# monahand1023/imageclust

Hardware: AMD Instinct MI355X
Metric: images/sec (embed+Ward) (higher is better)
Workload: dtype bf16; 1 GPU; the metric's size (configs[2]'s N=100000) on 1 GPU: 100000 synthetic 224x224x3 images (structured, seed 20250217; 100000 on this rank), ResNet50-v1 bf16 batch=256 -> 2048-d pooled E -> Ward min=5 max=50 (merge loop on GPU0) -> cluster ids on host; n_images_total=100000, embed_dim=2048, weights=synthetic seed 1, device=AMD Radeon Graphics (gfx950:sramecc+:xnack-)

## Files before the change

### imageclust_amd/_lib.py

```python
import ctypes as C
import os

import numpy as np

_HERE = os.path.dirname(os.path.abspath(__file__))
SO_PATH = os.environ.get("ICL_SO_PATH") or os.path.join(_HERE, "libimageclust_hip.so")

ICL_OK = 0
ICL_ERR_ARG, ICL_ERR_CONSTRAINT, ICL_ERR_HIP, ICL_ERR_NOMODEL, ICL_ERR_IO, ICL_ERR_UNSUPPORTED, ICL_ERR_OVERSIZE, ICL_ERR_NOMEM = range(1, 9)
HEAD_POOLED, HEAD_DENSE0 = 2048, 1000
PREC_FP32, PREC_BF16, PREC_BF16X3 = 0, 1, 2
UPDATE_EXACT, UPDATE_LW = 0, 1
SYNTH_NOISE, SYNTH_STRUCTURED = 0, 1
TILES_AUTO, TILES_LOCAL, TILES_DISTRIBUTED = 0, 1, 2
MERGE_GPU0, MERGE_SHARDED = 0, 1
CONV_P8_OFF, CONV_P8_AUTO, CONV_P8_ALL = 0, 1, 2
CONV_SPLIT = 16
ROWS_SINGLE, ROWS_EXACT_BATCH, ROWS_LW_BOUND, ROWS_LW_FAST, ROWS_SINGLE_APART = 0, 1, 2, 3, 4
FILE_FAIL_NEXT_LEADER = 0x100
MANY_MID_AUTO, MANY_MID_OFF, MANY_MID_ON = 0, 1, 2
PNG_HOST, PNG_GPU = 0, 1
ENTROPY_HOST, ENTROPY_GPU = 0, 1
K_CONV, K_DIST_EXACT, K_DIST_MFMA, K_ROWMIN, K_UPDATE, K_EMBED_OTHER, K_CONV64 = range(7)
K_NAMES = ["conv_igemm_kernel<*,128>", "ward_dist_exact_kernel", "dist_mfma_kernel", "row_argmin_*_kernel",
# ... 57 lines not shown
    ("icl_jpeg_coefs_mem", _int, [_vp, _vp, _vp, _i64, _int, _vp, _i64, _vp, _vp]),
    ("icl_jpeg_encode_bound", _i64, [_i32, _i32]),
    ("icl_jpeg_encode_rgb", _int, [_vp, _i32, _i32, _i32, _vp, _i64, _pi64]),
    ("icl_jpeg_encode_rgb_dev", _int, [_vp, _vp, _vp, _vp, _vp, _i64, _i32, _vp, _i32, _i64, _vp]),
    ("icl_downsize_image_file", _int, [C.c_char_p, _i64, _i32, _vp, _i64, _pi64, _vp]),
    ("icl_downsize_image_mem", _int, [_vp, _i64, _i64, _i32, _vp, _i64, _pi64, _vp]),
    ("icl_downsize_images", _int, [_vp, _vp, _i64, _i64, _i32, _i32, _vp, _i64, _vp, _vp]),
    ("icl_downsize_images_mem", _int, [_vp, _vp, _vp, _i64, _i64, _i32, _i32, _vp, _i64, _vp, _vp]),
    ("icl_last_downsize_stats", _int, [_vp, _pi64, _pi64, _pi64, _pi64, _pi64, _pi64, _vp]),
    ("icl_set_batch", _int, [_vp, _int]),
    ("icl_set_conv_options", _int, [_vp, _int]),
    ("icl_conv_stats", _int, [_vp, _vp, _vp]),
    ("icl_set_forward_prune", _int, [_vp, _int]),
    ("icl_forward_prune_stats", _int, [_vp, _vp]),
    ("icl_set_forward_prune_fused", _int, [_vp, _int]),
    ("icl_forward_prune_fused_stats", _int, [_vp, _vp]),
    ("icl_bottleneck56_sub", _int, [_vp, _vp, _int, _int, _int] + [_vp] * 9 + [_int, _int, _vp]),
    ("icl_conv1x1_mapped", _int, [_vp, _vp, _int, _int, _int, _int, _vp, _int, _vp, _vp, _vp, _int, _vp]),
    ("icl_conv_split_launches", _int, [_vp, _vp]),
    ("icl_conv2d_fused", _int, [_vp, _int, _vp, _int, _int, _int, _vp, _int, _int, _int, _int, _vp, _vp, _vp, _int, _vp]),
    ("icl_conv2d_dual", _int, [_vp, _int, _vp, _int, _int, _int, _vp, _vp, _int, _int, _vp, _int, _int, _vp, _vp, _int, _vp]),
    ("icl_embed_taps", _int, [_vp, _int, _vp, _int, _int, _vp]),
    ("icl_stem_pool", _int, [_vp, _int, _vp, _int, _vp]),
    ("icl_bottleneck56", _int, [_vp, _vp, _int, _int, _int, _int] + [_vp] * 13),
    ("icl_calc_optimal_clusters", _int, [_i64, _i64, _i64, _pi64]),
    ("icl_ward_distance_matrix", _int, [_vp, _vp, _vp, _i64, _i32, _vp, _i64]),
    ("icl_ward_distance_matrix_dev", _int, [_vp, _vp, _vp, _i64, _i32, _vp, _i64]),
    ("icl_merge_centroid", _int, [_vp, _vp, _i64, _vp, _i64, _i32, _vp]),
    ("icl_update_distance_matrix", _int, [_vp, _vp, _i64, _i64, _vp, _vp, _i32, _i64, _i64, _vp, _i64]),
    ("icl_find_closest", _int, [_vp, _vp, _i64, _i64, _pi64, _pi64]),
    ("icl_find_closest_dev", _int, [_vp, _vp, _i64, _i64, _pi64, _pi64]),
    ("icl_group_create", _int, [_pi32, _i32, C.POINTER(_vp)]),
    ("icl_group_destroy", None, [_vp]),
    ("icl_group_size", _i32, [_vp]),
    ("icl_group_ctx", _vp, [_vp, _i32]),
    ("icl_group_last_error", C.c_char_p, [_vp]),
    ("icl_group_load_onnx", _int, [_vp, C.c_char_p]),
    ("icl_group_load_blob", _int, [_vp, _vp, _i64]),
    ("icl_group_load_synthetic", _int, [_vp, C.c_uint64]),
    ("icl_group_embed_u8", _int, [_vp, _vp, _i64, _int, _int, _vp]),
    ("icl_group_cluster", _int, [_vp, _vp, _i64, _i32, _i32, _i32, _int, _vp, _vp, _pi32]),
    ("icl_set_ward_options", _int, [_vp, _int]),
    ("icl_embed_cluster_dev", _int, [_vp, _vp, _i64, _int, _i32, _i32, _int, _int, _vp, _vp, _vp, _pi32]),
    ("icl_group_embed_cluster", _int, [_vp, _vp, _i64, _int, _i32, _i32, _int, _vp, _vp, _vp, _pi32]),
    ("icl_ward_rows_partition", _int, [_i64, _i32, _i32, _pi64, _pi64]),
    ("icl_ward_span", _int, [_i64, _i64, _pi64, _pi64]),
# ... 473 lines not shown
        a, b = C.c_int64(0), C.c_int64(0)
        check(self.h, self.L.icl_conv_stats(self.h, C.byref(a), C.byref(b)))
        return a.value, b.value

    def conv_split_launches(self):
        a = C.c_int64(0)
        check(self.h, self.L.icl_conv_split_launches(self.h, C.byref(a)))
        return a.value

    def set_conv_options(self, p8_mode=1):
        check(self.h, self.L.icl_set_conv_options(self.h, p8_mode))

    def set_forward_prune(self, on=True):
        check(self.h, self.L.icl_set_forward_prune(self.h, 1 if on else 0))

    def forward_prune_stats(self):
        a = C.c_int64(0)
        check(self.h, self.L.icl_forward_prune_stats(self.h, C.byref(a)))
        return a.value

    def set_forward_prune_fused(self, on=True):
        check(self.h, self.L.icl_set_forward_prune_fused(self.h, 1 if on else 0))

    def forward_prune_fused_stats(self):
        a = C.c_int64(0)
        check(self.h, self.L.icl_forward_prune_fused_stats(self.h, C.byref(a)))
        return a.value

    def embed_u8(self, imgs, head=HEAD_POOLED, prec=PREC_FP32):
        imgs = np.ascontiguousarray(imgs, np.uint8).reshape(-1, IMG_BYTES)
        n = imgs.shape[0]
        out = np.empty((n, head), np.float32)
        check(self.h, self.L.icl_embed_u8(self.h, imgs.ctypes.data, n, head, prec, out.ctypes.data))
        return out

    def embed_u8_dev(self, d_imgs, n, d_out, head=HEAD_POOLED, prec=PREC_BF16):
        check(self.h, self.L.icl_embed_u8_dev(self.h, _vp(d_imgs), n, head, prec, _vp(d_out)))

    def embed_file(self, path, head=HEAD_DENSE0):
        out = np.empty(head, np.float32)
        check(self.h, self.L.icl_embed_file(self.h, os.fsencode(path), head, out.ctypes.data))
        return out

    def _files_call(self, fn, paths, *args):
        enc = [os.fsencode(p) for p in paths]
        arr = (C.c_char_p * max(1, len(enc)))(*enc)
# ... 242 lines not shown

    def conv2d_dual(self, x_nhwc, w1, x2_nhwc, w2, stride2, scale, shift, relu=True, prec=PREC_FP32):
        f = lambda a: np.ascontiguousarray(a, np.float32)
        x, x2, w1, w2, sc, sh = f(x_nhwc), f(x2_nhwc), f(w1), f(w2), f(scale), f(shift)
        B, Ho, _, Cin = x.shape
        _, H2, _, Cin2 = x2.shape
        Cout = w1.shape[0]
        assert x2.shape[0] == B and w1.shape == (Cout, Cin) and w2.shape == (Cout, Cin2) and sc.shape == (Cout,) and sh.shape == (Cout,)
        y = np.empty((B, Ho, Ho, Cout), np.float32)
        check(self.h, self.L.icl_conv2d_dual(self.h, prec, x.ctypes.data, B, Ho, Cin, w1.ctypes.data, x2.ctypes.data, H2, Cin2, w2.ctypes.data,
                                             int(stride2), Cout, sc.ctypes.data, sh.ctypes.data, 1 if relu else 0, y.ctypes.data))
        return y

    def embed_taps(self, imgs, tap, prec=PREC_FP32):
        a = np.ascontiguousarray(imgs, np.uint8).reshape(-1, IMG_BYTES)
        out = np.empty((a.shape[0],) + tap_shape(tap), np.float32)
        check(self.h, self.L.icl_embed_taps(self.h, prec, a.ctypes.data, a.shape[0], int(tap), out.ctypes.data))
        return out

    def stem_pool(self, imgs, prec=PREC_FP32):
        a = np.ascontiguousarray(imgs, np.uint8).reshape(-1, IMG_BYTES)
        out = np.empty((a.shape[0], 56, 56, 64), np.float32)
        check(self.h, self.L.icl_stem_pool(self.h, prec, a.ctypes.data, a.shape[0], out.ctypes.data))
        return out

    def bottleneck56(self, x_nhwc, w1, bn1, w2_oihw, bn2, w3, bn3, wds=None, bnds=None):
        f = lambda a: np.ascontiguousarray(a, np.float32)
        x = f(x_nhwc)
        B, H, W, Cin = x.shape
        y = np.empty((B, H, W, 256), np.float32)
        keep = [x, f(w1), f(bn1[0]), f(bn1[1]), f(w2_oihw), f(bn2[0]), f(bn2[1]), f(w3), f(bn3[0]), f(bn3[1])]
        keep += [None, None, None] if wds is None else [f(wds), f(bnds[0]), f(bnds[1])]
        ptr = [None if a is None else a.ctypes.data for a in keep]
        check(self.h, self.L.icl_bottleneck56(self.h, ptr[0], B, H, W, Cin, *ptr[1:], y.ctypes.data))
        return y

    def bottleneck56_sub(self, x_nhwc, w1, bn1, w2_oihw, bn2, w3, bn3, sub, fill):
        f = lambda a: np.ascontiguousarray(a, np.float32)
        x = f(x_nhwc)
        B, H, W, Cin = x.shape
        assert Cin == 256
        y = np.empty((B, H, W, 256), np.float32)
        keep = [x, f(w1), f(bn1[0]), f(bn1[1]), f(w2_oihw), f(bn2[0]), f(bn2[1]), f(w3), f(bn3[0]), f(bn3[1])]
        ptr = [a.ctypes.data for a in keep]
        check(self.h, self.L.icl_bottleneck56_sub(self.h, ptr[0], B, H, W, *ptr[1:], int(sub), int(fill), y.ctypes.data))
        return y
# ... 750 lines not shown
```

### imageclust_amd/csrc/icl_common.h

```cpp
#pragma once
#include <hip/hip_runtime.h>

#include <condition_variable>
#include <cstdarg>
#include <cstdint>
#include <cstdio>
#include <functional>
#include <mutex>
#include <string>
#include <vector>

#include "../../include/icl_model_format.h"
#include "../../include/imageclust.h"

#define ICL_MAXF 3.40282346638528859811704183484516925e+38f

struct icl_ctx;
int icl_fail(icl_ctx *ctx, int code, const char *fmt, ...);
static inline hipStream_t icl_main_stream(const icl_ctx *ctx);

#define ICL_HIP(ctx, call)                                                                                     \
    do {                                                                                                       \
        hipError_t e__ = (call);                                                                               \
        if (e__ != hipSuccess)                                                                                 \
// ... 126 lines not shown
    void *file_batcher = nullptr;
    icl_dev_grow many;
    int many_mid = 0;
    int64_t many_stats[4] = {0, 0, 0, 0};
    icl_ingest_ws *ingest = nullptr;
    ingest_totals ingest_last;
    int entropy_mode = 0;
    int png_mode = 0;
    icl_requests_ws *requests = nullptr;
    double requests_ms[3] = {0, 0, 0};
    icl_jenc_ws *jenc = nullptr;
    dz_totals downsize_last;
    icl_dev_grow nearest;
    int nearest_splits = 0;
    int64_t nearest_stats[4] = {0, 0, 0, 0};
    icl_dev_grow pairs;
    int64_t pairs_stats[4] = {0, 0, 0, 0};
    icl_dev_grow fit;
    int64_t fit_stats[4] = {0, 0, 0, 0};
    int64_t between_stats[5] = {0, 0, 0, 0, 0};
    std::vector<const void *> lds_optin;
    int fwd_prune_fused = 1;
    int64_t pruned_fused = 0;
};

static inline hipStream_t icl_main_stream(const icl_ctx *ctx) { return ctx->stream; }

struct icl_device_guard {
    int prev = -1;
    bool ok = true;
    explicit icl_device_guard(int dev)
    {
        if (hipGetDevice(&prev) != hipSuccess) prev = -1;
        if (prev != dev) ok = (hipSetDevice(dev) == hipSuccess);
    }
    ~icl_device_guard()
    {
        if (prev >= 0) (void)hipSetDevice(prev);
    }
};

struct icl_prof_scope {
    icl_ctx *c;
    int k;
    hipEvent_t a = nullptr, b = nullptr;
    icl_prof_scope(icl_ctx *ctx, int kclass, double flops, double bytes);
// ... 108 lines not shown
```

### imageclust_amd/csrc/icl_core.hip

```cpp
#include "icl_common.h"

#include <cstring>

static thread_local std::string g_tls_err;

int icl_fail(icl_ctx *ctx, int code, const char *fmt, ...)
{
    char buf[1024];
    va_list ap;
    va_start(ap, fmt);
    vsnprintf(buf, sizeof buf, fmt, ap);
    va_end(ap);
    if (ctx) ctx->err = buf;
    g_tls_err = buf;
    return code;
}

extern "C" const char *icl_version(void) { return "imageclust_hip 0.1 (gfx950)"; }

extern "C" const char *icl_last_error(icl_ctx *ctx) { return ctx ? ctx->err.c_str() : g_tls_err.c_str(); }

extern "C" int icl_create(int device, icl_ctx **out)
{
    if (!out) return icl_fail(nullptr, ICL_ERR_ARG, "icl_create: out is NULL");
// ... 179 lines not shown
{
    if (!ctx || !pruned_blocks) return icl_fail(ctx, ICL_ERR_ARG, "icl_forward_prune_stats: NULL argument");
    std::lock_guard<std::mutex> lk(ctx->mu);
    *pruned_blocks = ctx->pruned_blocks;
    return ICL_OK;
}

extern "C" int icl_set_forward_prune_fused(icl_ctx *ctx, int on)
{
    if (!ctx || on < 0 || on > 1) return icl_fail(ctx, ICL_ERR_ARG, "icl_set_forward_prune_fused: on must be 0 or 1");
    std::lock_guard<std::mutex> lk(ctx->mu);
    ctx->fwd_prune_fused = on;
    return ICL_OK;
}

extern "C" int icl_forward_prune_fused_stats(icl_ctx *ctx, int64_t *pruned_launches)
{
    if (!ctx || !pruned_launches) return icl_fail(ctx, ICL_ERR_ARG, "icl_forward_prune_fused_stats: NULL argument");
    std::lock_guard<std::mutex> lk(ctx->mu);
    *pruned_launches = ctx->pruned_fused;
    return ICL_OK;
}

extern "C" int icl_conv_split_launches(icl_ctx *ctx, int64_t *launches)
{
    if (!ctx || !launches) return icl_fail(ctx, ICL_ERR_ARG, "icl_conv_split_launches: NULL argument");
    std::lock_guard<std::mutex> lk(ctx->mu);
    *launches = ctx->conv_sk_launches;
    return ICL_OK;
}

extern "C" int icl_conv_stats(icl_ctx *ctx, int64_t *p8_launches, int64_t *other_launches)
{
    if (!ctx) return icl_fail(ctx, ICL_ERR_ARG, "icl_conv_stats: ctx is NULL");
    std::lock_guard<std::mutex> lk(ctx->mu);
    if (p8_launches) *p8_launches = ctx->conv_launches[0];
    if (other_launches) *other_launches = ctx->conv_launches[1];
    return ICL_OK;
}

static hipEvent_t take_event(icl_ctx *c)
{
    if (!c->event_pool.empty()) {
        hipEvent_t e = c->event_pool.back();
        c->event_pool.pop_back();
        return e;
// ... 114 lines not shown
```

### imageclust_amd/csrc/resnet.hip

```cpp
#include "icl_common.h"
#include "mfma_tile.h"
#include "resnet_model.h"

#include <algorithm>
#include <cmath>
#include <cstring>
#include <deque>
#include <new>
#include <thread>
#include <type_traits>
#include <vector>

#include "conv_select.h"
static_assert(CONV_PREC_FP32 == ICL_PREC_FP32 && CONV_PREC_BF16 == ICL_PREC_BF16 && CONV_PREC_BF16X3 == ICL_PREC_BF16X3 && CONV_TILE_M == CV_BM && CONV_ROW_BYTES == CV_ROWB,
              "conv_select.h restates these constants");

#include "resnet_fused.h"
#include "conv_p8.h"
#include "conv_wr.h"

template <typename T, int BN>
struct conv_resid {
    static constexpr int NPASS = 64 / (256 / (BN / T::KE));
    uint4 v[2][NPASS];
// ... 613 lines not shown
            const float4 wv = *reinterpret_cast<const float4 *>(W + (int64_t)o * nin + i);
            s += xv.x * wv.x + xv.y * wv.y + xv.z * wv.z + xv.w * wv.w;
        }
#pragma unroll
        for (int off = 32; off > 0; off >>= 1) s += __shfl_down(s, off, 64);
        if (lane == 0) y[b * nout + o] = s + bias[o];
    }
}

template <typename T, int BN, bool DUAL, bool EARLY>
static void launch_conv_igemm(icl_ctx *ctx, const conv_args &a, const conv_choice &c)
{
    icl_lds_optin(ctx, (const void *)conv_igemm_kernel<T, BN, DUAL, 2, EARLY>, (int)conv_igemm_lds(BN, 2));
    hipLaunchKernelGGL((conv_igemm_kernel<T, BN, DUAL, 2, EARLY>), dim3(c.blocks), dim3(c.threads), c.lds, ctx->cur_stream ? ctx->cur_stream : ctx->stream, a);
}

struct fwd_env {
    int conv_mode, wr_pt256, fuse;
};
static const fwd_env &forward_env()
{
    static const fwd_env e = [] {
        const char *m = getenv("ICL_CONV_MODE"), *p = getenv("ICL_WR_PT256"), *f = getenv("ICL_FUSE");
        return fwd_env{m ? atoi(m) : 1, p && atoi(p) == 32 ? 32 : 64, f ? atoi(f) : 15};
    }();
    return e;
}
static int fuse_mask() { return forward_env().fuse; }
static conv_opts conv_opts_of(const icl_ctx *ctx)
{
    const fwd_env &e = forward_env();
    return conv_opts{ctx->conv_p8, ctx->conv_wr, ctx->conv_sk, ctx->conv_sk_min_k, e.conv_mode, e.wr_pt256, ctx->prop.multiProcessorCount};
}

template <typename T>
static int launch_conv_t(icl_ctx *ctx, int prec, const conv_args &real, const conv_choice &c)
{
    constexpr bool X3 = is_x3<T>::value;
    if (c.family == CONV_UNSUPPORTED) return icl_fail(ctx, ICL_ERR_UNSUPPORTED, "%s", c.why);
    conv_args a = conv_kernel_view(prec, real);
    a.gx = c.gx;
    a.gy = c.gy;
    icl_prof_scope ps(ctx, a.Cout % 128 == 0 ? ICL_K_CONV : ICL_K_CONV64, 2.0 * (double)real.M * real.Cout * real.K, 0.0);
    bool split = false;
    switch (c.family) {
    case CONV_WR:
        launch_conv_wr(ctx, a, c);
// ... 129 lines not shown
    if (!ctx || !x || !w || !scale || !shift || !y || B < 1 || H < 1 || sub < 1 || Cin < 1 || Cout < 1)
        return icl_fail(ctx, ICL_ERR_ARG, "icl_conv1x1_mapped: bad argument");
    if ((int64_t)B * H * H * Cout * 2 >= (1LL << 31)) return icl_fail(ctx, ICL_ERR_UNSUPPORTED, "icl_conv1x1_mapped: the full tensor exceeds the kernel's 32-bit buffer offsets");
    return run_entry(ctx, "icl_conv1x1_mapped", false, y, [&](entry_io &io) -> int {
        const int prec = ICL_PREC_BF16;
        const prune_map pm = prune_map_make(sub, H, H);
        const size_t nx = (size_t)B * pm.Ho * pm.Wo * Cin, ny = (size_t)B * H * H * Cout;
        dev_guard &dx = io.buf(), &dw = io.buf(), &dr = io.buf(), &dy = io.buf(), &dz = io.buf(), &dsc = io.buf(), &dsh = io.buf();
        ICL_TRY(upload_as(ctx, prec, &dx.p, x, nx));
        ICL_TRY(zero_page(ctx, "icl_conv1x1_mapped", dz));
        ICL_TRY(upload_as(ctx, prec, &dw.p, w, (size_t)Cout * Cin));
        if (residual) ICL_TRY(upload_as(ctx, prec, &dr.p, residual, ny));
        ICL_TRY(upload_as(ctx, prec, &dy.p, y, ny));
        ICL_TRY(upload_as(ctx, ICL_PREC_FP32, &dsc.p, scale, (size_t)Cout));
        ICL_TRY(upload_as(ctx, ICL_PREC_FP32, &dsh.p, shift, (size_t)Cout));
        conv_args a = conv_plain(dx.p, dw.p, dy.p, dr.p, (const float *)dsc.p, (const float *)dsh.p, dz.p, B, pm.Ho, Cin, Cout, 1, 1, 0, relu);
        a.omap = pm;
        io.returns(prec, dy.p, ny);
        if (conv_select(prec, a, conv_opts_of(ctx)).family != CONV_WR) return icl_fail(ctx, ICL_ERR_UNSUPPORTED, "icl_conv1x1_mapped: Cin = %d, Cout = %d is no shape of the streaming kernel's mapped form", Cin, Cout);
        return launch_conv_prec(ctx, prec, a);
    });
}

static int stem_per_cu(int prec, int fuse)
{
    const size_t cu_lds = (size_t)160 * 1024;
    if (prec == ICL_PREC_BF16 && (fuse & 1) && (fuse & 8)) return std::max<int>(1, std::min<int>(5, (int)(cu_lds / stem2_lds_bytes())));
    if (prec == ICL_PREC_BF16X3 || (fuse & 1)) return std::max<int>(1, (int)(cu_lds / (prec == ICL_PREC_BF16 ? stem_pool_lds_bytes<BF16>() : stem_pool_lds_bytes<F32>())));
    return std::max<int>(1, (int)(cu_lds / (prec == ICL_PREC_BF16 ? stem_lds_bytes<BF16>() : stem_lds_bytes<F32>())));
}
static fwd_opts forward_opts_of(const icl_ctx *ctx, int prec)
{
    return fwd_opts{conv_opts_of(ctx), fuse_mask(), ctx->fwd_prune, stem_per_cu(prec, fuse_mask()), ctx->fwd_prune_fused};
}

template <typename T>
static void launch_stem_pool(icl_ctx *ctx, int prec, const uint8_t *d_img, int B, void *pooled, unsigned grid, hipStream_t strm)
{
    icl_model *m = ctx->model;
    if (prec == ICL_PREC_BF16 && (fuse_mask() & 8)) {
        const conv_layer &L0 = m->conv[0];
        icl_prof_scope ps(ctx, ICL_K_CONV64, 2.0 * (double)B * 112 * 112 * 64 * 147, 0.0);
        const int nunits = B * SP_STRIPS;
        hipLaunchKernelGGL(stem2_pool_kernel, dim3(grid), dim3(256), stem2_lds_bytes(), strm, d_img, (const uint16_t *)L0.wfold, L0.shift, (uint16_t *)pooled, nunits);
        return;
    }
    constexpr bool SPLIT = is_x3<T>::value;
    typedef typename std::conditional<SPLIT, F32, T>::type TS;
    icl_lds_optin(ctx, (const void *)stem_pool_kernel<TS, SPLIT>, (int)stem_pool_lds_bytes<TS>());
    const conv_args a = conv_stem(m, m->conv[0].w[SPLIT ? ICL_PREC_FP32 : prec], pooled, B, B * SP_STRIPS * SP_TILES);
    icl_prof_scope ps(ctx, ICL_K_CONV64, 2.0 * (double)a.M * 64 * 147, 0.0);
    const int nunits = B * SP_STRIPS;
    hipLaunchKernelGGL((stem_pool_kernel<TS, SPLIT>), dim3(grid), dim3(256), stem_pool_lds_bytes<TS>(), strm, d_img, a, nunits);
}

static int launch_bneck56_args(icl_ctx *ctx, bneck_args &a, bool ds, int sub, hipStream_t strm)
{
    if (sub != 1 && (sub != 2 || ds)) return icl_fail(ctx, ICL_ERR_UNSUPPORTED, "fused bottleneck: no kernel for sub = %d%s", sub, ds ? " with a downsample branch" : "");
    const int B = a.B;
    if ((int64_t)B * a.H * a.W * 512 >= (1LL << 31)) return icl_fail(ctx, ICL_ERR_UNSUPPORTED, "fused bottleneck: batch of %d images exceeds the 32-bit buffer offsets", B);
    bneck56_grid(B, a.W, ctx->prop.multiProcessorCount, &a.nstrips, &a.ngroups);
#ifdef BN56_TIMERS
    static unsigned long long *dbg = nullptr;
    if (!dbg) (void)hipMalloc((void **)&dbg, 16 * 8);
    a.dbg = dbg;
#endif
    const double px = (double)B * a.H * a.W, px23 = (double)B * prune_extent(a.H, sub) * prune_extent(a.W, sub);
// ... 47 lines not shown
{
    const icl_model *m = ctx->model;
    icl_conv_rec recs[ICL_RESNET50_NCONV];
    for (int i = 0; i < m->nconv; ++i) recs[i] = m->conv[i].rec;
    *plan = forward_make_plan(recs, m->nconv, prec, B, head == ICL_HEAD_DENSE0, tap, forward_opts_of(ctx, prec));
    if (plan->err) return icl_fail(ctx, ICL_ERR_UNSUPPORTED, "forward pass, convolution %d (cin=%d cout=%d k=%d): %s", plan->err_layer, recs[plan->err_layer].cin, recs[plan->err_layer].cout, recs[plan->err_layer].k, plan->err);
    return ICL_OK;
}

template <typename T>
static int forward_batch(icl_ctx *ctx, int prec, const fwd_plan &plan, const uint8_t *d_img, int head, float *d_out, int lane, hipStream_t strm)
{
    typedef typename T::elem elem;
    icl_model *m = ctx->model;
    ctx->cur_stream = strm;
    const int B = plan.B;
    void *const *buf = m->buf[lane];
    float *pooled = head == ICL_HEAD_POOLED ? d_out : m->pooled[lane];
    for (const fwd_step &s : plan.steps) {
        const conv_layer &L = m->conv[s.layer];
        switch (s.kind) {
        case FWD_STEM2_POOL:
        case FWD_STEM_POOL:
            launch_stem_pool<T>(ctx, prec, d_img, B, buf[s.y], s.blocks, strm);
            break;
        case FWD_STEM:
            if constexpr (!is_x3<T>::value) {
                icl_lds_optin(ctx, (const void *)stem_conv_kernel<T>, (int)stem_lds_bytes<T>());
                const conv_args a = conv_stem(m, L.w[prec], buf[s.y], B, B * 98);
                icl_prof_scope ps(ctx, ICL_K_CONV64, 2.0 * (double)a.M * 64 * 147, 0.0);
                hipLaunchKernelGGL((stem_conv_kernel<T>), dim3(s.blocks), dim3(s.threads), stem_lds_bytes<T>(), strm, d_img, a);
            }
            break;
        case FWD_MAXPOOL:
            if constexpr (!is_x3<T>::value) {
                icl_prof_scope ps(ctx, ICL_K_EMBED_OTHER, 0.0, (double)B * (802816.0 + 200704.0) * sizeof(elem));
                hipLaunchKernelGGL((maxpool_kernel<T>), dim3(s.blocks), dim3(s.threads), 0, strm, (const elem *)buf[s.x], B, 112, 64, (elem *)buf[s.y]);
            }
            break;
        case FWD_BNECK56:
            ICL_TRY(launch_bneck56(ctx, L, m->conv[s.layer + 1], m->conv[s.layer + 2], s.ds ? &m->conv[s.layer + 3] : nullptr, buf[s.x], buf[s.y], B, s.sub, strm));
            ctx->pruned_fused += s.sub == 2;
            break;
        case FWD_CONV: {
            conv_args a = s.a;
            a.X = buf[s.x]; a.Y = buf[s.y]; a.R = s.r != FWD_NONE ? buf[s.r] : nullptr; a.zero = m->zero;
            if (s.ds) {
                a.Wt = L.wfused[prec]; a.scale = m->ones; a.shift = L.shift_fused; a.X2 = buf[s.x2];
            } else {
                a.Wt = L.w[prec]; a.scale = L.scale; a.shift = L.shift;
            }
            ICL_TRY(launch_conv_t<T>(ctx, prec, a, s.c));
            ctx->pruned_blocks += s.pruned;
            break;
        }
        case FWD_AVGPOOL: {
            icl_prof_scope ps(ctx, ICL_K_EMBED_OTHER, 0.0, (double)B * 49.0 * 2048.0 * (is_x3<T>::value ? 4 : sizeof(elem)));
            hipLaunchKernelGGL((avgpool_kernel<T>), dim3(s.blocks), dim3(s.threads), 0, strm, (const elem *)buf[s.x], B, 49, ICL_FEAT_DIM, pooled, (int64_t)ICL_FEAT_DIM);
            break;
        }
        default: {
            icl_prof_scope ps(ctx, ICL_K_EMBED_OTHER, 2.0 * B * 2048.0 * 1000.0, 0.0);
            hipLaunchKernelGGL(fc_kernel, dim3(s.blocks), dim3(s.threads), 0, strm, pooled, m->fcw, m->fcb, B, ICL_FEAT_DIM, ICL_FC_OUT, d_out);
        }
        }
    }
    ICL_HIP(ctx, hipGetLastError());
    return ICL_OK;
}

extern "C" int icl_stem_pool(icl_ctx *ctx, int prec, const uint8_t *img, int B, float *out)
{
    if (!ctx || !img || !out || B < 1) return icl_fail(ctx, ICL_ERR_ARG, "icl_stem_pool: bad argument");
    if (!prec_ok(prec)) return icl_fail(ctx, ICL_ERR_ARG, "bad prec");
    return run_entry(ctx, "icl_stem_pool", true, out, [&](entry_io &io) -> int {
        const size_t ny = (size_t)B * 56 * 56 * 64;
        dev_guard &dimg = io.buf(), &dy = io.buf();
        ICL_TRY(icl_dev_alloc(ctx, dimg, (size_t)B * ICL_IMG_BYTES, "icl_stem_pool: images"));
        ICL_TRY(icl_dev_alloc(ctx, dy, ny * prec_act_bytes(prec), "icl_stem_pool: output"));
        if (hipMemcpy(dimg.p, img, (size_t)B * ICL_IMG_BYTES, hipMemcpyHostToDevice) != hipSuccess) return icl_fail(ctx, ICL_ERR_HIP, "icl_stem_pool: upload");
        const unsigned grid = fwd_stem_blocks((int64_t)B * SP_STRIPS, stem_per_cu(prec, fuse_mask() | 1), ctx->prop.multiProcessorCount);
        with_prec(prec, [&](auto t) { launch_stem_pool<decltype(t)>(ctx, prec, (const uint8_t *)dimg.p, B, dy.p, grid, ctx->stream); });
        io.returns(prec, dy.p, ny);
        const hipError_t e = hipGetLastError();
        return e == hipSuccess ? ICL_OK : icl_fail(ctx, ICL_ERR_HIP, "icl_stem_pool: %s", hipGetErrorString(e));
    });
}

static int bottleneck56_entry(icl_ctx *ctx, const float *x, int B, int H, int W, int Cin, const float *w1, const float *sc1, const float *sh1,
                              const float *w2, const float *sc2, const float *sh2, const float *w3, const float *sc3, const float *sh3,
                              const float *wds, const float *scds, const float *shds, int sub, const uint16_t *fill, float *y)
{
    if (!ctx || !x || !w1 || !sc1 || !sh1 || !w2 || !sc2 || !sh2 || !w3 || !sc3 || !sh3 || !y || B < 1 || H < 1 || W < 1)
        return icl_fail(ctx, ICL_ERR_ARG, "icl_bottleneck56: bad argument");
    const bool has_ds = wds != nullptr;
    if (has_ds && (!scds || !shds)) return icl_fail(ctx, ICL_ERR_ARG, "icl_bottleneck56: downsample scale / shift missing");
    if (Cin != (has_ds ? 64 : 256)) return icl_fail(ctx, ICL_ERR_UNSUPPORTED, "icl_bottleneck56: Cin must be 256 (identity) or 64 (downsample branch)");
    if ((int64_t)B * H * W * 512 >= (1LL << 31)) return icl_fail(ctx, ICL_ERR_UNSUPPORTED, "icl_bottleneck56: tensor exceeds the kernel's 32-bit buffer offsets");
    return run_entry(ctx, "icl_bottleneck56", false, y, [&](entry_io &io) -> int {
        const size_t nx = (size_t)B * H * W * Cin, ny = (size_t)B * H * W * 256;
        std::vector<float> f1, p2, f2, f3, fds, f3ds, h3(sh3, sh3 + 256);
        pack_row_scale(w1, sc1, 64, Cin, f1);
        pack_ohwi(w2, 64, 64, 3, p2);
        pack_row_scale(p2.data(), sc2, 64, 576, f2);
        pack_row_scale(w3, sc3, 256, 64, f3);
        if (has_ds) {
            pack_row_scale(wds, scds, 256, 64, fds);
            pack_row_concat(f3.data(), 64, fds.data(), 64, 256, f3ds);
            for (int co = 0; co < 256; ++co) h3[(size_t)co] = sh3[co] + shds[co];
// ... 194 lines not shown
```

### imageclust_amd/csrc/resnet_fused.h

```cpp
#pragma once
#include "conv_select.h"
#include "mfma_tile.h"
#include "resnet_model.h"

typedef float f32x4 __attribute__((ext_vector_type(4)));

__device__ __forceinline__ f32x4 mfma16(const uint4 &a, const uint4 &b, const f32x4 &c)
{
    return __builtin_amdgcn_mfma_f32_16x16x32_bf16(__builtin_bit_cast(bf16x8_t, a), __builtin_bit_cast(bf16x8_t, b), c, 0, 0, 0);
}
typedef unsigned u32x4_t __attribute__((ext_vector_type(4)));
typedef int i32x4_t __attribute__((ext_vector_type(4)));
#define BN56_OOB 0x80000000u
__device__ __forceinline__ i32x4_t bn56_srd(const void *base, unsigned bytes)
{
    const unsigned long long a = (unsigned long long)base;
    i32x4_t r;
    r.x = (int)(unsigned)a;
    r.y = (int)(unsigned)(a >> 32);
    r.z = (int)bytes;
    r.w = 0x00020000;
    return r;
}
__device__ __forceinline__ void bload_lds16_asm(const i32x4_t &srd, unsigned voff, unsigned soff, unsigned lds_dst)
{
    unsigned keep;
// ... 366 lines not shown
            for (int kh = 0; kh < 3; ++kh) {
                const int rr = 2 * pr + kh;
                if (rr == 0 && t == 0) continue;
                const unsigned char *rowp = rr == 0 ? carry_cur : ptile + (rr - 1) * 2048;
#pragma unroll
                for (int kw = 0; kw < 3; ++kw) {
                    const int ci = 2 * pc + kw;
                    if (s == 0 && ci == 0) continue;
                    const uint4 rawv = *reinterpret_cast<const uint4 *>(rowp + ci * 128 + (((ch ^ (ci >> 1)) & 7) << 4));
                    best[0] = __builtin_elementwise_max(best[0], __builtin_bit_cast(i16x2_t, rawv.x));
                    best[1] = __builtin_elementwise_max(best[1], __builtin_bit_cast(i16x2_t, rawv.y));
                    best[2] = __builtin_elementwise_max(best[2], __builtin_bit_cast(i16x2_t, rawv.z));
                    best[3] = __builtin_elementwise_max(best[3], __builtin_bit_cast(i16x2_t, rawv.w));
                }
            }
            const uint4 o = make_uint4(__builtin_bit_cast(uint32_t, best[0]), __builtin_bit_cast(uint32_t, best[1]), __builtin_bit_cast(uint32_t, best[2]),
                                       __builtin_bit_cast(uint32_t, best[3]));
            *reinterpret_cast<uint4 *>(Yg + ((b * 56 + 4 * t + pr) * 56 + 7 * s + pc) * 64 + ch * 8) = o;
        }
        if (!has_next) break;
        unit = nu;
        t = nt;
        __syncthreads();
    }
}

#ifdef BN56_TIMERS
#define BN56_STAMP(k)                                                                              \
    do {                                                                                           \
        unsigned long long t__;                                                                    \
        __builtin_amdgcn_sched_barrier(0);                                                         \
        asm volatile("s_memtime %0\n\ts_waitcnt lgkmcnt(0)" : "=s"(t__)::"memory");                \
        __builtin_amdgcn_sched_barrier(0);                                                         \
        tacc[k] += t__ - tlast;                                                                    \
        tlast = t__;                                                                               \
    } while (0)
#define BN56_TIMER_DECL unsigned long long tacc[8] = {0, 0, 0, 0, 0, 0, 0, 0}, tlast = 0
#define BN56_TIMER_START asm volatile("s_memtime %0\n\ts_waitcnt lgkmcnt(0)" : "=s"(tlast)::"memory")
#define BN56_TIMER_FLUSH(role)                                                                     \
    if (p.dbg && blockIdx.x == 0 && w == 0 && lane == 0)                                            \
        for (int k__ = 0; k__ < 8; ++k__) p.dbg[(role)*8 + k__] = tacc[k__]
#define BN56_FRONT_SEGMENTS {"carry+conv1", "wait E", "dma+t1 epi", "wait C", "conv2+t2 epi", "wait x", "wait D", ""}
#define BN56_BACK_SEGMENTS {"t2 + side reads", "MFMAs + epilogue", "read-back + stores", "barrier waits", "", "", "", ""}
#else
#define BN56_STAMP(k)
#define BN56_TIMER_DECL
// ... 404 lines not shown
```

### include/imageclust.h

```cpp
#ifndef IMAGECLUST_H
#define IMAGECLUST_H
#include <stdint.h>

#ifdef __cplusplus
extern "C" {
#endif

typedef struct icl_ctx icl_ctx;

enum {
    ICL_OK = 0,
    ICL_ERR_ARG = 1,
    ICL_ERR_CONSTRAINT = 2,
    ICL_ERR_HIP = 3,
    ICL_ERR_NOMODEL = 4,
    ICL_ERR_IO = 5,
    ICL_ERR_UNSUPPORTED = 6,
    ICL_ERR_OVERSIZE = 7,
    ICL_ERR_NOMEM = 8
};

enum { ICL_HEAD_POOLED = 2048,
       ICL_HEAD_DENSE0 = 1000   };
enum { ICL_PREC_FP32 = 0,
// ... 41 lines not shown
int icl_last_ingest_stats(icl_ctx *ctx, int64_t *gpu_jpegs, int64_t *host_files, int64_t *upload_bytes,
                          double *host_decode_s);
enum { ICL_ENTROPY_HOST = 0, ICL_ENTROPY_GPU = 1 };
int icl_set_ingest_options(icl_ctx *ctx, int entropy_mode);
int icl_last_entropy_stats(icl_ctx *ctx, int64_t *gpu_entropy_jpegs, int64_t *host_entropy_jpegs, int64_t *redone_on_host,
                           int64_t *stream_bytes);
int icl_jpeg_coefs_files(icl_ctx *ctx, const char *const *paths, int64_t n, int entropy_mode, int16_t *coefs, int64_t cap,
                         int64_t *offsets , int32_t *state );
int icl_jpeg_coefs_file_host(const char *path, int sub_bits, int16_t *coefs, int64_t cap, int64_t *need, int32_t *info );
enum { ICL_PNG_HOST = 0, ICL_PNG_GPU = 1 };
int icl_set_png_options(icl_ctx *ctx, int png_mode);
int icl_last_png_stats(icl_ctx *ctx, int64_t *gpu_pngs, int64_t *host_pngs, int64_t *redone_on_host, int64_t *stream_bytes);
int icl_png_raw_files(icl_ctx *ctx, const char *const *paths, int64_t n, int stage, uint8_t *raw, int64_t cap, int64_t *offsets ,
                      int32_t *state );
int icl_png_raw_file_host(const char *path, int stage, uint8_t *raw, int64_t cap, int64_t *need, int32_t *info );
int icl_png_raw_mem_host(const uint8_t *data, int64_t bytes, int stage, uint8_t *raw, int64_t cap, int64_t *need, int32_t *info );
int icl_set_batch(icl_ctx *ctx, int batch);
enum { ICL_CONV_P8_OFF = 0, ICL_CONV_P8_AUTO = 1, ICL_CONV_P8_ALL = 2, ICL_CONV_SPLIT = 16 };
int icl_set_conv_options(icl_ctx *ctx, int p8_mode);
int icl_set_forward_prune(icl_ctx *ctx, int on);
int icl_forward_prune_stats(icl_ctx *ctx, int64_t *pruned_blocks);
int icl_set_forward_prune_fused(icl_ctx *ctx, int on);
int icl_forward_prune_fused_stats(icl_ctx *ctx, int64_t *pruned_launches);
int icl_conv_split_launches(icl_ctx *ctx, int64_t *launches);
int icl_conv_stats(icl_ctx *ctx, int64_t *p8_launches, int64_t *other_launches);
int icl_conv2d_fused(icl_ctx *ctx, int prec, const float *x, int B, int H, int Cin, const float *w, int Cout, int k,
                     int stride, int pad, const float *scale, const float *shift, const float *residual, int relu,
                     float *y);

int icl_conv2d_dual(icl_ctx *ctx, int prec, const float *x, int B, int Ho, int Cin, const float *w1, const float *x2, int H2, int Cin2,
                    const float *w2, int stride2, int Cout, const float *scale, const float *shift, int relu, float *y);
int icl_conv1x1_mapped(icl_ctx *ctx, const float *x, int B, int H, int sub, int Cin, const float *w, int Cout, const float *scale,
                       const float *shift, const float *residual, int relu, float *y);
int icl_embed_taps(icl_ctx *ctx, int prec, const uint8_t *hwc_rgb, int B, int tap, float *out);

int icl_stem_pool(icl_ctx *ctx, int prec, const uint8_t *hwc_rgb, int B, float *out);
int icl_bottleneck56(icl_ctx *ctx, const float *x, int B, int H, int W, int Cin, const float *w1, const float *sc1, const float *sh1,
                     const float *w2, const float *sc2, const float *sh2, const float *w3, const float *sc3, const float *sh3,
                     const float *wds, const float *scds, const float *shds, float *y);
int icl_bottleneck56_sub(icl_ctx *ctx, const float *x, int B, int H, int W, const float *w1, const float *sc1, const float *sh1,
                         const float *w2, const float *sc2, const float *sh2, const float *w3, const float *sc3, const float *sh3,
                         int sub, int fill, float *y);

typedef struct icl_group icl_group;
int icl_group_create(const int32_t *devices, int32_t ndev, icl_group **out);
void icl_group_destroy(icl_group *g);
int32_t icl_group_size(icl_group *g);
icl_ctx *icl_group_ctx(icl_group *g, int32_t i);
const char *icl_group_last_error(icl_group *g);
int icl_group_load_onnx(icl_group *g, const char *path);
int icl_group_load_blob(icl_group *g, const void *blob, int64_t bytes);
int icl_group_load_synthetic(icl_group *g, uint64_t seed);
int icl_group_embed_u8(icl_group *g, const uint8_t *hwc_rgb, int64_t n, int head, int prec, float *out);
int icl_group_cluster(icl_group *g, const float *E, int64_t n, int32_t d, int32_t min_size, int32_t max_size, int update,
                      int32_t *cluster_id, int32_t *member_rank, int32_t *n_clusters);
int icl_group_embed_cluster(icl_group *g, const uint8_t *hwc_rgb, int64_t n, int prec, int32_t min_size, int32_t max_size, int update,
                            float *E_out, int32_t *cluster_id, int32_t *member_rank, int32_t *n_clusters);

enum { ICL_TILES_AUTO = 0, ICL_TILES_LOCAL = 1, ICL_TILES_DISTRIBUTED = 2 };
// ... 195 lines not shown
```

Before: 76030 images/sec.

## Add ring-buffered stem conv+pool kernel reusing overlapping input rows across tiles

Adds a new stem3 kernel that keeps a circular LDS buffer of converted bf16 image rows. Each successive tile along an image loads only the 16 new rows instead of refetching the full 21-row patch. It prefetches the next tile's pixels while the MFMA stem convolution runs, then does the 3x3 maxpool in registers with DPP row shifts. The default fuse mask goes from 15 to 31, which turns the ring path on, and the blocks per CU now come from an occupancy query. The kernel carries considerably more complex indexing and halo-handling logic, with a risk of boundary errors or lower occupancy.

```diff
diff --git a/imageclust_amd/_lib.py b/imageclust_amd/_lib.py
--- a/imageclust_amd/_lib.py
+++ b/imageclust_amd/_lib.py
@@ -103,6 +103,8 @@
     ("icl_conv2d_dual", _int, [_vp, _int, _vp, _int, _int, _int, _vp, _vp, _int, _int, _vp, _int, _int, _vp, _vp, _int, _vp]),
     ("icl_embed_taps", _int, [_vp, _int, _vp, _int, _int, _vp]),
     ("icl_stem_pool", _int, [_vp, _int, _vp, _int, _vp]),
+    ("icl_stem_pool_form", _int, [_vp, _int, _vp, _int, _int, _vp]),
+    ("icl_set_forward_stem_ring", _int, [_vp, _int]),
     ("icl_bottleneck56", _int, [_vp, _vp, _int, _int, _int, _int] + [_vp] * 13),
     ("icl_calc_optimal_clusters", _int, [_i64, _i64, _i64, _pi64]),
     ("icl_ward_distance_matrix", _int, [_vp, _vp, _vp, _i64, _i32, _vp, _i64]),
@@ -622,6 +624,9 @@
     def set_forward_prune_fused(self, on=True):
         check(self.h, self.L.icl_set_forward_prune_fused(self.h, 1 if on else 0))
 
+    def set_forward_stem_ring(self, on=True):
+        check(self.h, self.L.icl_set_forward_stem_ring(self.h, 1 if on else 0))
+
     def forward_prune_fused_stats(self):
         a = C.c_int64(0)
         check(self.h, self.L.icl_forward_prune_fused_stats(self.h, C.byref(a)))
@@ -910,6 +915,12 @@
         a = np.ascontiguousarray(imgs, np.uint8).reshape(-1, IMG_BYTES)
         out = np.empty((a.shape[0], 56, 56, 64), np.float32)
         check(self.h, self.L.icl_stem_pool(self.h, prec, a.ctypes.data, a.shape[0], out.ctypes.data))
+        return out
+
+    def stem_pool_form(self, imgs, form, grid=0):
+        a = np.ascontiguousarray(imgs, np.uint8).reshape(-1, IMG_BYTES)
+        out = np.empty((a.shape[0], 56, 56, 64), np.float32)
+        check(self.h, self.L.icl_stem_pool_form(self.h, int(form), a.ctypes.data, a.shape[0], int(grid), out.ctypes.data))
         return out
 
     def bottleneck56(self, x_nhwc, w1, bn1, w2_oihw, bn2, w3, bn3, wds=None, bnds=None):
diff --git a/imageclust_amd/csrc/icl_common.h b/imageclust_amd/csrc/icl_common.h
--- a/imageclust_amd/csrc/icl_common.h
+++ b/imageclust_amd/csrc/icl_common.h
@@ -172,6 +172,8 @@
     std::vector<const void *> lds_optin;
     int fwd_prune_fused = 1;
     int64_t pruned_fused = 0;
+    int fwd_stem_ring = -1;
+    int stem3_per_cu = 0;
 };
 
 static inline hipStream_t icl_main_stream(const icl_ctx *ctx) { return ctx->stream; }
diff --git a/imageclust_amd/csrc/icl_core.hip b/imageclust_amd/csrc/icl_core.hip
--- a/imageclust_amd/csrc/icl_core.hip
+++ b/imageclust_amd/csrc/icl_core.hip
@@ -225,6 +225,14 @@
     return ICL_OK;
 }
 
+extern "C" int icl_set_forward_stem_ring(icl_ctx *ctx, int on)
+{
+    if (!ctx || on < 0 || on > 1) return icl_fail(ctx, ICL_ERR_ARG, "icl_set_forward_stem_ring: on must be 0 or 1");
+    std::lock_guard<std::mutex> lk(ctx->mu);
+    ctx->fwd_stem_ring = on;
+    return ICL_OK;
+}
+
 extern "C" int icl_conv_split_launches(icl_ctx *ctx, int64_t *launches)
 {
     if (!ctx || !launches) return icl_fail(ctx, ICL_ERR_ARG, "icl_conv_split_launches: NULL argument");
diff --git a/imageclust_amd/csrc/resnet.hip b/imageclust_amd/csrc/resnet.hip
--- a/imageclust_amd/csrc/resnet.hip
+++ b/imageclust_amd/csrc/resnet.hip
@@ -659,7 +659,7 @@
 {
     static const fwd_env e = [] {
         const char *m = getenv("ICL_CONV_MODE"), *p = getenv("ICL_WR_PT256"), *f = getenv("ICL_FUSE");
-        return fwd_env{m ? atoi(m) : 1, p && atoi(p) == 32 ? 32 : 64, f ? atoi(f) : 15};
+        return fwd_env{m ? atoi(m) : 1, p && atoi(p) == 32 ? 32 : 64, f ? atoi(f) : 31};
     }();
     return e;
 }
@@ -835,27 +835,42 @@
     });
 }
 
-static int stem_per_cu(int prec, int fuse)
+static bool stem_ring_on(const icl_ctx *ctx) { return ctx->fwd_stem_ring < 0 ? (fuse_mask() & 16) != 0 : ctx->fwd_stem_ring != 0; }
+static int stem3_per_cu(icl_ctx *ctx)
+{
+    if (ctx->stem3_per_cu <= 0) {
+        int n = 0;
+        if (hipOccupancyMaxActiveBlocksPerMultiprocessor(&n, stem3_pool_kernel, 256, stem3_lds_bytes()) != hipSuccess) {
+            (void)hipGetLastError();
+            n = 0;
+        }
+        ctx->stem3_per_cu = std::max(1, std::min(n, 8));
+    }
+    return ctx->stem3_per_cu;
+}
+static int stem_per_cu(icl_ctx *ctx, int prec, int fuse, bool ring)
 {
     const size_t cu_lds = (size_t)160 * 1024;
+    if (prec == ICL_PREC_BF16 && (fuse & 1) && (fuse & 8) && ring) return stem3_per_cu(ctx);
     if (prec == ICL_PREC_BF16 && (fuse & 1) && (fuse & 8)) return std::max<int>(1, std::min<int>(5, (int)(cu_lds / stem2_lds_bytes())));
     if (prec == ICL_PREC_BF16X3 || (fuse & 1)) return std::max<int>(1, (int)(cu_lds / (prec == ICL_PREC_BF16 ? stem_pool_lds_bytes<BF16>() : stem_pool_lds_bytes<F32>())));
     return std::max<int>(1, (int)(cu_lds / (prec == ICL_PREC_BF16 ? stem_lds_bytes<BF16>() : stem_lds_bytes<F32>())));
 }
-static fwd_opts forward_opts_of(const icl_ctx *ctx, int prec)
-{
-    return fwd_opts{conv_opts_of(ctx), fuse_mask(), ctx->fwd_prune, stem_per_cu(prec, fuse_mask()), ctx->fwd_prune_fused};
+static fwd_opts forward_opts_of(icl_ctx *ctx, int prec)
+{
+    return fwd_opts{conv_opts_of(ctx), fuse_mask(), ctx->fwd_prune, stem_per_cu(ctx, prec, fuse_mask(), stem_ring_on(ctx)), ctx->fwd_prune_fused};
 }
 
 template <typename T>
-static void launch_stem_pool(icl_ctx *ctx, int prec, const uint8_t *d_img, int B, void *pooled, unsigned grid, hipStream_t strm)
+static void launch_stem_pool(icl_ctx *ctx, int prec, const uint8_t *d_img, int B, void *pooled, unsigned grid, hipStream_t strm, bool ring)
 {
     icl_model *m = ctx->model;
     if (prec == ICL_PREC_BF16 && (fuse_mask() & 8)) {
         const conv_layer &L0 = m->conv[0];
         icl_prof_scope ps(ctx, ICL_K_CONV64, 2.0 * (double)B * 112 * 112 * 64 * 147, 0.0);
         const int nunits = B * SP_STRIPS;
-        hipLaunchKernelGGL(stem2_pool_kernel, dim3(grid), dim3(256), stem2_lds_bytes(), strm, d_img, (const uint16_t *)L0.wfold, L0.shift, (uint16_t *)pooled, nunits);
+        if (ring) hipLaunchKernelGGL(stem3_pool_kernel, dim3(grid), dim3(256), stem3_lds_bytes(), strm, d_img, (const uint16_t *)L0.wfold, L0.shift, (uint16_t *)pooled, nunits);
+        else hipLaunchKernelGGL(stem2_pool_kernel, dim3(grid), dim3(256), stem2_lds_bytes(), strm, d_img, (const uint16_t *)L0.wfold, L0.shift, (uint16_t *)pooled, nunits);
         return;
     }
     constexpr bool SPLIT = is_x3<T>::value;
@@ -949,7 +964,7 @@
         switch (s.kind) {
         case FWD_STEM2_POOL:
         case FWD_STEM_POOL:
-            launch_stem_pool<T>(ctx, prec, d_img, B, buf[s.y], s.blocks, strm);
+            launch_stem_pool<T>(ctx, prec, d_img, B, buf[s.y], s.blocks, strm, stem_ring_on(ctx));
             break;
         case FWD_STEM:
             if constexpr (!is_x3<T>::value) {
@@ -996,22 +1011,34 @@
     return ICL_OK;
 }
 
-extern "C" int icl_stem_pool(icl_ctx *ctx, int prec, const uint8_t *img, int B, float *out)
-{
-    if (!ctx || !img || !out || B < 1) return icl_fail(ctx, ICL_ERR_ARG, "icl_stem_pool: bad argument");
-    if (!prec_ok(prec)) return icl_fail(ctx, ICL_ERR_ARG, "bad prec");
-    return run_entry(ctx, "icl_stem_pool", true, out, [&](entry_io &io) -> int {
+static int stem_pool_entry(icl_ctx *ctx, const char *who, int prec, int form, const uint8_t *img, int B, int grid, float *out)
+{
+    return run_entry(ctx, who, true, out, [&](entry_io &io) -> int {
         const size_t ny = (size_t)B * 56 * 56 * 64;
         dev_guard &dimg = io.buf(), &dy = io.buf();
         ICL_TRY(icl_dev_alloc(ctx, dimg, (size_t)B * ICL_IMG_BYTES, "icl_stem_pool: images"));
         ICL_TRY(icl_dev_alloc(ctx, dy, ny * prec_act_bytes(prec), "icl_stem_pool: output"));
-        if (hipMemcpy(dimg.p, img, (size_t)B * ICL_IMG_BYTES, hipMemcpyHostToDevice) != hipSuccess) return icl_fail(ctx, ICL_ERR_HIP, "icl_stem_pool: upload");
-        const unsigned grid = fwd_stem_blocks((int64_t)B * SP_STRIPS, stem_per_cu(prec, fuse_mask() | 1), ctx->prop.multiProcessorCount);
-        with_prec(prec, [&](auto t) { launch_stem_pool<decltype(t)>(ctx, prec, (const uint8_t *)dimg.p, B, dy.p, grid, ctx->stream); });
+        if (hipMemcpy(dimg.p, img, (size_t)B * ICL_IMG_BYTES, hipMemcpyHostToDevice) != hipSuccess) return icl_fail(ctx, ICL_ERR_HIP, "%s: upload", who);
+        const bool ring = form < 0 ? stem_ring_on(ctx) : form == 1;
+        const int fuse = form < 0 ? fuse_mask() | 1 : 9;
+        const unsigned g = grid > 0 ? (unsigned)grid : fwd_stem_blocks((int64_t)B * SP_STRIPS, stem_per_cu(ctx, prec, fuse, ring), ctx->prop.multiProcessorCount);
+        with_prec(prec, [&](auto t) { launch_stem_pool<decltype(t)>(ctx, prec, (const uint8_t *)dimg.p, B, dy.p, g, ctx->stream, ring); });
         io.returns(prec, dy.p, ny);
         const hipError_t e = hipGetLastError();
-        return e == hipSuccess ? ICL_OK : icl_fail(ctx, ICL_ERR_HIP, "icl_stem_pool: %s", hipGetErrorString(e));
+        return e == hipSuccess ? ICL_OK : icl_fail(ctx, ICL_ERR_HIP, "%s: %s", who, hipGetErrorString(e));
     });
+}
+extern "C" int icl_stem_pool(icl_ctx *ctx, int prec, const uint8_t *img, int B, float *out)
+{
+    if (!ctx || !img || !out || B < 1) return icl_fail(ctx, ICL_ERR_ARG, "icl_stem_pool: bad argument");
+    if (!prec_ok(prec)) return icl_fail(ctx, ICL_ERR_ARG, "bad prec");
+    return stem_pool_entry(ctx, "icl_stem_pool", prec, -1, img, B, 0, out);
+}
+extern "C" int icl_stem_pool_form(icl_ctx *ctx, int form, const uint8_t *img, int B, int grid, float *out)
+{
+    if (!ctx || !img || !out || B < 1 || form < 0 || form > 1 || grid < 0) return icl_fail(ctx, ICL_ERR_ARG, "icl_stem_pool_form: bad argument (form 0 or 1, grid >= 0)");
+    if (!(fuse_mask() & 8)) return icl_fail(ctx, ICL_ERR_UNSUPPORTED, "icl_stem_pool_form: ICL_FUSE without bit 3 has no bf16-patch stem");
+    return stem_pool_entry(ctx, "icl_stem_pool_form", ICL_PREC_BF16, form, img, B, grid, out);
 }
 
 static int bottleneck56_entry(icl_ctx *ctx, const float *x, int B, int H, int W, int Cin, const float *w1, const float *sc1, const float *sh1,
diff --git a/imageclust_amd/csrc/resnet_fused.h b/imageclust_amd/csrc/resnet_fused.h
--- a/imageclust_amd/csrc/resnet_fused.h
+++ b/imageclust_amd/csrc/resnet_fused.h
@@ -2,6 +2,7 @@
 #include "conv_select.h"
 #include "mfma_tile.h"
 #include "resnet_model.h"
+#include "stem_ring_map.h"
 
 typedef float f32x4 __attribute__((ext_vector_type(4)));
 
@@ -414,6 +415,137 @@
         unit = nu;
         t = nt;
         __syncthreads();
+    }
+}
+
+static_assert(ST3_PW == ST2_PW && ST3_PH == STEM_PH && ST3_NEW * SP_TILES == ST3_IMG, "stem_ring_map.h restates the stem's geometry");
+static constexpr size_t stem3_lds_bytes() { return (size_t)ST3_RING * ST3_PW * 8; }
+
+__device__ __forceinline__ uint32_t st3_row_shl(uint32_t v, int n)
+{
+    return n == 1 ? (uint32_t)__builtin_amdgcn_update_dpp(0, (int)v, 0x101, 0xf, 0xf, true) : (uint32_t)__builtin_amdgcn_update_dpp(0, (int)v, 0x102, 0xf, 0xf, true);
+}
+__device__ __forceinline__ uint32_t st3_pk_max(uint32_t a, uint32_t b)
+{
+    return __builtin_bit_cast(uint32_t, __builtin_elementwise_max(__builtin_bit_cast(i16x2_t, a), __builtin_bit_cast(i16x2_t, b)));
+}
+
+__global__ __launch_bounds__(256) void stem3_pool_kernel(const uint8_t *__restrict__ img, const uint16_t *__restrict__ W2k ,
+                                                        const float *__restrict__ shift, uint16_t *__restrict__ Yg , int nunits)
+{
+    extern __shared__ __attribute__((aligned(16))) unsigned char smem[];
+    unsigned char *ring = smem;
+    const int tid = threadIdx.x, lane = tid & 63;
+    const int w = __builtin_amdgcn_readfirstlane(tid >> 6);
+    const int r16 = lane & 15, q = lane >> 4;
+    uint4 wr[7];
+#pragma unroll
+    for (int kh = 0; kh < 7; ++kh) wr[kh] = *reinterpret_cast<const uint4 *>(W2k + (size_t)(16 * w + r16) * ST2_K + 32 * kh + 8 * q);
+    const float4 hf = *reinterpret_cast<const float4 *>(shift + 16 * w + 4 * q);
+    const f32x4 hv = f32x4{hf.x, hf.y, hf.z, hf.w};
+    const unsigned boff = (unsigned)((2 * r16 + 2 * q) * 8);
+    const float sc255 = (float)(1.0 / 255.0);
+    uint32_t px[3];
+    int fg = 0;
+    unsigned frow = 0;
+    bool fvalid = false;
+    auto fetch = [&](int unit, int t) {
+        int pr;
+        fvalid = st3_fetch_role(tid, t, &pr, &fg);
+        const int iy = st3_image_row(t, pr), x0 = st3_group_x(unit & 7, fg);
+        const bool in = fvalid && st3_row_in_image(iy) && st3_group_in_image(x0);
+        const uint32_t *p = reinterpret_cast<const uint32_t *>(img + (int64_t)(unit >> 3) * (int64_t)ICL_IMG_BYTES + iy * 672 + x0 * 3);
+        px[0] = in ? p[0] : 0u;
+        px[1] = in ? p[1] : 0u;
+        px[2] = in ? p[2] : 0u;
+        frow = (unsigned)(st3_ring_row(t, fvalid ? pr : 0) * (ST3_PW * 8));
+    };
+    auto convert_store = [&]() {
+        if (!fvalid) return;
+        uint2 o[4];
+#pragma unroll
+        for (int e = 0; e < 4; ++e) {
+            uint32_t c[3];
+#pragma unroll
+            for (int k = 0; k < 3; ++k) {
+                const int byte = 3 * e + k;
+                c[k] = (uint32_t)BF16::from_f((float)((px[byte >> 2] >> (8 * (byte & 3))) & 0xffu) * sc255);
+            }
+            o[e] = make_uint2(c[0] | (c[1] << 16), c[2]);
+        }
+        unsigned char *dst = ring + frow + st3_group_pixel(fg, 0) * 8;
+        if (st3_group_lead_kept(fg)) {
+            *reinterpret_cast<uint2 *>(dst) = o[0];
+            *reinterpret_cast<uint4 *>(dst + 8) = make_uint4(o[1].x, o[1].y, o[2].x, o[2].y);
+        }
+        if (st3_group_last_kept(fg)) *reinterpret_cast<uint2 *>(dst + 24) = o[3];
+    };
+    int unit = blockIdx.x, t = 0;
+    if (unit >= nunits) return;
+    fetch(unit, 0);
+    __builtin_amdgcn_s_waitcnt(0x0f70);
+    convert_store();
+    __syncthreads();
+    uint2 prev = make_uint2(0u, 0u);
+    int rb = 0;
+    for (;;) {
+        int nt = t + 1, nu = unit;
+        if (nt == SP_TILES) {
+            nt = 0;
+            nu = unit + (int)gridDim.x;
+        }
+        const bool has_next = nu < nunits;
+        if (has_next) fetch(nu, nt);
+        f32x4 acc[8];
+#pragma unroll
+        for (int r = 0; r < STEM_PH; ++r) {
+            int row = rb + r;
+            if (row >= ST3_RING) row -= ST3_RING;
+            const uint4 bf = *reinterpret_cast<const uint4 *>(ring + row * (ST3_PW * 8) + boff);
+#pragma unroll
+            for (int m = 0; m < 8; ++m) {
+                const int kh = r - 2 * m;
+                if (kh >= 0 && kh < 7) acc[m] = mfma16(wr[kh], bf, kh == 0 ? hv : acc[m]);
+            }
+        }
+        __builtin_amdgcn_sched_barrier(0);
+        __builtin_amdgcn_s_waitcnt(0x0f70);
+        if (has_next) {
+            if (nt == 0) __syncthreads();
+            convert_store();
+        }
+        {
+            const int s = unit & 7;
+            const int64_t b = unit >> 3;
+            uint2 o[8];
+#pragma unroll
+            for (int m = 0; m < 8; ++m) {
+                o[m].x = pack_relu_bf16x2(acc[m][0], acc[m][1]);
+                o[m].y = pack_relu_bf16x2(acc[m][2], acc[m][3]);
+            }
+            const bool nocol = s == 0 && r16 == 0;
+            const bool st = (r16 & 1) == 0 && r16 <= 12;
+            uint16_t *yo = Yg + ((b * 56 + 4 * t) * 56 + 7 * s + (r16 >> 1)) * 64 + 16 * w + 4 * q;
+#pragma unroll
+            for (int pr = 0; pr < 4; ++pr) {
+                const uint2 up = pr == 0 ? prev : o[2 * pr - 1];
+                uint2 v;
+                v.x = st3_pk_max(st3_pk_max(up.x, o[2 * pr].x), o[2 * pr + 1].x);
+                v.y = st3_pk_max(st3_pk_max(up.y, o[2 * pr].y), o[2 * pr + 1].y);
+                v.x = nocol ? 0u : v.x;
+                v.y = nocol ? 0u : v.y;
+                uint2 h;
+                h.x = st3_pk_max(st3_pk_max(v.x, st3_row_shl(v.x, 1)), st3_row_shl(v.x, 2));
+                h.y = st3_pk_max(st3_pk_max(v.y, st3_row_shl(v.y, 1)), st3_row_shl(v.y, 2));
+                if (st) *reinterpret_cast<uint2 *>(yo + pr * (56 * 64)) = h;
+            }
+            prev = nt == 0 ? make_uint2(0u, 0u) : o[7];
+        }
+        if (!has_next) break;
+        __syncthreads();
+        unit = nu;
+        t = nt;
+        rb = nt == 0 ? 0 : (rb + ST3_NEW >= ST3_RING ? rb + ST3_NEW - ST3_RING : rb + ST3_NEW);
     }
 }
 
diff --git a/imageclust_amd/csrc/stem_ring_map.h b/imageclust_amd/csrc/stem_ring_map.h
--- /dev/null
+++ b/imageclust_amd/csrc/stem_ring_map.h
@@ -0,0 +1,33 @@
+#pragma once
+
+#ifdef __HIPCC__
+#define ST3_FI __host__ __device__ __forceinline__
+#else
+#define ST3_FI inline
+#endif
+
+#define ST3_IMG 224
+#define ST3_PH 21
+#define ST3_NEW 16
+#define ST3_RING 37
+#define ST3_PW 40
+#define ST3_USED 38
+#define ST3_GROUPS 11
+
+ST3_FI int st3_ring_row(int t, int pr) { return (ST3_NEW * t + pr) % ST3_RING; }
+ST3_FI int st3_image_row(int t, int pr) { return ST3_NEW * t - 3 + pr; }
+ST3_FI int st3_first_new_row(int t) { return t == 0 ? 0 : ST3_PH - ST3_NEW; }
+ST3_FI int st3_new_rows(int t) { return t == 0 ? ST3_PH : ST3_NEW; }
+ST3_FI bool st3_fetch_role(int tid, int t, int *pr, int *g)
+{
+    const int slot = tid / ST3_GROUPS;
+    *g = tid - slot * ST3_GROUPS;
+    *pr = st3_first_new_row(t) + slot;
+    return slot < st3_new_rows(t);
+}
+ST3_FI int st3_group_x(int s, int g) { return 28 * s - 8 + 4 * g; }
+ST3_FI int st3_group_pixel(int g, int e) { return 4 * g - 3 + e; }
+ST3_FI bool st3_group_lead_kept(int g) { return g > 0; }
+ST3_FI bool st3_group_last_kept(int g) { return g < ST3_GROUPS - 1; }
+ST3_FI bool st3_row_in_image(int iy) { return (unsigned)iy < (unsigned)ST3_IMG; }
+ST3_FI bool st3_group_in_image(int x0) { return (unsigned)x0 < (unsigned)ST3_IMG; }
diff --git a/include/imageclust.h b/include/imageclust.h
--- a/include/imageclust.h
+++ b/include/imageclust.h
@@ -87,6 +87,7 @@
 int icl_forward_prune_stats(icl_ctx *ctx, int64_t *pruned_blocks);
 int icl_set_forward_prune_fused(icl_ctx *ctx, int on);
 int icl_forward_prune_fused_stats(icl_ctx *ctx, int64_t *pruned_launches);
+int icl_set_forward_stem_ring(icl_ctx *ctx, int on);
 int icl_conv_split_launches(icl_ctx *ctx, int64_t *launches);
 int icl_conv_stats(icl_ctx *ctx, int64_t *p8_launches, int64_t *other_launches);
 int icl_conv2d_fused(icl_ctx *ctx, int prec, const float *x, int B, int H, int Cin, const float *w, int Cout, int k,
@@ -100,6 +101,7 @@
 int icl_embed_taps(icl_ctx *ctx, int prec, const uint8_t *hwc_rgb, int B, int tap, float *out);
 
 int icl_stem_pool(icl_ctx *ctx, int prec, const uint8_t *hwc_rgb, int B, float *out);
+int icl_stem_pool_form(icl_ctx *ctx, int form, const uint8_t *hwc_rgb, int B, int grid, float *out);
 int icl_bottleneck56(icl_ctx *ctx, const float *x, int B, int H, int W, int Cin, const float *w1, const float *sc1, const float *sh1,
                      const float *w2, const float *sc2, const float *sh2, const float *w3, const float *sc3, const float *sh3,
                      const float *wds, const float *scds, const float *shds, float *y);
```

After: 76360 images/sec, median of 6. No clear change (+0.4%).
